# tspooner/rl_markets

Measured on AMD Instinct MI355X. Metric: env-steps/sec (whole node) at 65 536 parallel books, higher is better.
Workload: dtype f64

## Files before the change

### rl_markets_amd/csrc/lob_engine.hip

```cpp
#define LOB_TU_SPLIT 1
#define LOB_TU_MAIN 1
#include <hip/hip_runtime.h>
#include <math.h>
#include <stdio.h>
#include <stdlib.h>
#include <string.h>

#include <algorithm>
#include <climits>
#include <condition_variable>
#include <initializer_list>
#include <map>
#include <mutex>
#include <string>
#include <system_error>
#include <thread>
#include <vector>

#include "lob_internal.h"
#include "lob_fast.h"
#include "lob_kernels.h"
#include "lob_launch.h"

#define HIPCHK(expr)                                                                         \
// ... 8 lines not shown
#define LOB_PS(e) (const DevParams*)(e)->P_dev, (e)->S.self

#define LOB_HINT_RING 64
#define LOB_HINT_LAG 16
#define LOB_HINT_EVERY 8

struct KTimer {
    std::vector<std::pair<hipEvent_t, hipEvent_t>> pending;
    double total_ms = 0.0;
    int64_t launches = 0;
};

struct Switches {
    bool no_memo = false, no_carry = false, no_combine = false, light = true, force_fuse_act = false, t_light = true, no_fuse = false;
    bool q_pair = true, dq_pair = true, trace_lanes_off = false, acc_fuse = true, rest_merge = true, acc_dense = true;
    int q_lanes = -1, force_general = -1;
    int env_lanes = 0, env16_max = 4096;
    int acc_batches = 0, acc_shift = -1;
    int cb_slots = 0, ow_slots = 0, amb_cap = 0, cbd_ids = 0;
    int track_ring = 4096, track_refill = 64;
    long long upload_piece_recs = 0, spx_count = 0;
    bool upload_pinned = true;
    bool fuse_act = true, inline_general = true, env_step = true, prepass_roles = false, sarsa_lanes_off = false, dq_fast_off = false;
    bool rest_side = true, acc_block = true, exp_learn_first = false, no_hint = false;
    int env_step_lanes = 64, reset_lanes = 64, n_groups = 1, acc_reps = 0, ts_lds = 0, ts_grid = 0;
};

struct EnginePlan {
    int groups = 1;
    bool combine = false, memo = false, carry_verdicts = false, sarsa_lanes = false;
    bool q_lanes = false;
    bool q_pair = false;
    bool t_light = false;
    bool fuse = false;
    bool fused_act_ok = false;
    bool env_step = false, half_waves = false, env16 = false;
    bool inline_ok = false;
    int env_lanes = 64;
    bool acc_block_ok = false;
    bool dense_ids = false;
    bool acc_fuse_ok = false;
    bool rest_side_ok = false;
    bool learn_first = false;
};

struct lob_engine {
    int device = 0;
    int B = 0;
    lob_params params;
    Switches sw;
    EnginePlan plan;
    DevParams P;
    DevParams* P_dev = nullptr;
    DevState S;
    DevState* S_dev = nullptr;
    DevState S_pushed;
    hipStream_t stream = nullptr;
    hipStream_t stream2 = nullptr;
    hipEvent_t ev_fork = nullptr, ev_join = nullptr, ev_stagger = nullptr;
    hipEvent_t ev_rest_go = nullptr, ev_rest_done = nullptr;
    long long flow[8] = {0, 0, 0, 0, 0, 0, 0, 0};
    long long hint_reads = 0, hint_misses = 0;
    bool dense_ever = false;
    u64* rest_hint = nullptr;
    u64* rest_hint_dev = nullptr;
    hipEvent_t hint_ev[LOB_HINT_RING] = {};
    long long hint_step = 0;
    unsigned long long hint_serial = 0;
    uint32_t hint_tags[LOB_HINT_RING] = {};
    int hint_now = 0;
    int rest_recent = 0;
    int reg_apar = 0;
    int td_parity = 0;
    int step_id = 0;
    int list_par = 0;
    int last_par = 0;
// ... 178 lines not shown
bool env_is(const char* n, char c) { const char* g = getenv(n); return g && g[0] == c; }
long long env_in(const char* n, long long lo, long long hi, long long dflt) { const char* g = getenv(n); const long long v = g ? atoll(g) : dflt; return v >= lo && v <= hi ? v : dflt; }
int env_one_of(const char* n, std::initializer_list<int> allowed, int dflt) {
    const char* g = getenv(n);
    for (int a : allowed) if (g && atoi(g) == a) return a;
    return dflt;
}
int env_pow2(const char* n, int lo, int hi, int dflt) { const int v = (int)env_in(n, lo, hi, dflt); return (v & (v - 1)) == 0 ? v : dflt; }

Switches read_switches() {
    Switches s;
    s.no_memo = env_is("LOB_NO_MEMO", '1'); s.no_carry = env_is("LOB_NO_CARRY", '1'); s.no_combine = env_is("LOB_NO_COMBINE", '1');
    s.light = !env_is("LOB_NO_LIGHT", '1'); s.force_fuse_act = env_is("LOB_FUSE_ACT", '1');
    s.t_light = !env_is("LOB_NO_TLIGHT", '1'); s.no_fuse = env_is("LOB_NO_FUSE", '1');
    s.q_pair = !env_is("LOB_Q_PAIR", '0'); s.dq_pair = !env_is("LOB_DQ_PAIR", '0'); s.trace_lanes_off = env_is("LOB_TRACE_LANES", '0');
    s.acc_fuse = !env_is("LOB_ACC_FUSE", '0'); s.rest_merge = !env_is("LOB_REST_MERGE", '0'); s.acc_dense = !env_is("LOB_ACC_DENSE", '0');
    s.q_lanes = env_set("LOB_Q_LANES") ? (env_is("LOB_Q_LANES", '1') ? 1 : 0) : -1;
    s.force_general = env_is("LOB_MOSTLY_GENERAL", '1') ? 1 : env_is("LOB_MOSTLY_GENERAL", '0') ? 0 : -1;
    const bool exps = lobk_experiments() != 0;
    s.env_lanes = exps ? env_one_of("LOB_ENV_LANES", {16, 32, 64, 256}, 0) : env_one_of("LOB_ENV_LANES", {16, 64}, 0);
    s.env16_max = (int)env_in("LOB_ENV16_MAX", 0, INT_MAX, s.env16_max);
    s.acc_batches = env_one_of("LOB_ACC_BATCHES", {1, 2, 4, 8}, 0);
    const int acc_lanes = env_one_of("LOB_ACC_LANES", {8, 16, 32, 64}, 0);
    s.acc_shift = acc_lanes ? __builtin_ctz(acc_lanes) : -1;
    s.cb_slots = env_pow2("LOB_CB_SLOTS", 64, 1 << 24, 0); s.ow_slots = env_pow2("LOB_OW_SLOTS", 64, 1 << 26, 0);
    s.amb_cap = (int)env_in("LOB_AMB_CAP", 1, 1 << 18, 0); s.cbd_ids = (int)env_in("LOB_CBD_IDS", 8, LOB_CBD_CAP, 0);
    s.track_ring = env_pow2("LOB_TRACK_RING", 256, 1 << 20, s.track_ring); s.track_refill = (int)env_in("LOB_TRACK_REFILL", 1, INT_MAX, s.track_refill);
    s.upload_piece_recs = env_in("LOB_UPLOAD_PIECE_RECS", 1, LLONG_MAX, 0); s.upload_pinned = !env_is("LOB_UPLOAD_PINNED", '0');
    s.spx_count = env_in("LOB_SPX_COUNT", 64, LLONG_MAX, 0);
    if (!exps) return s;
// ... 6 lines not shown
    s.ts_lds = (int)env_in("LOB_TS_LDS", INT_MIN, INT_MAX, 0); s.ts_grid = (int)env_in("LOB_TS_GRID", INT_MIN, INT_MAX, 0);
    return s;
}

EnginePlan plan_paths(const DevParams& P, int B, int n_cus, const Switches& sw) {
    EnginePlan pl;
    const bool sarsa = P.algo == LOB_ALGO_SARSA, ql = P.algo == LOB_ALGO_QLAMBDA, dq = P.algo == LOB_ALGO_DOUBLE_Q;
    pl.groups = B >= 1024 ? sw.n_groups : 1;
    pl.combine = !P.theta_private && !sw.no_combine;
    pl.env_lanes = sw.env_lanes ? sw.env_lanes : (B <= 16384 ? 16 : 64);
    pl.fused_act_ok = sw.light && sw.fuse_act && sw.env_lanes == 0 && (B >= 1024 || sw.force_fuse_act);
    pl.env_step = P.T <= 2 && sw.env_step;
    pl.half_waves = sw.env_step_lanes == 32 && pl.env_step && !dq;
    pl.inline_ok = pl.env_step && sw.inline_general && !pl.half_waves;
    pl.env16 = !dq && B <= sw.env16_max && P.D <= 16 && P.Wd <= 64;
    pl.q_lanes = sw.q_lanes >= 0 ? sw.q_lanes == 1 : (long long)B >= (long long)LOB_QL_BLOCK * n_cus / 2;
    pl.q_pair = sw.q_pair && P.M < (1ll << 27) && (!dq || sw.dq_pair);
    pl.t_light = (ql || dq) && sw.t_light;
    pl.fuse = pl.t_light && pl.q_lanes && !sw.no_fuse;
    pl.memo = !P.theta_private && !P.r_learn && sw.n_groups == 1 && !sw.no_memo;
    if (dq) pl.memo = pl.memo && pl.fuse && pl.fused_act_ok && pl.env_step && pl.combine && P.trace_gens == 32 && !sw.dq_fast_off;
    pl.carry_verdicts = !P.theta_private && !sw.no_carry && !pl.memo;
    pl.sarsa_lanes = pl.memo && pl.combine && P.trace_gens == 32 && !sw.sarsa_lanes_off && !sw.trace_lanes_off && (sarsa || pl.fuse);
    pl.acc_block_ok = sw.acc_block && pl.memo && B >= 4 * LOB_ACB_BLOCK;
    pl.dense_ids = pl.acc_block_ok && pl.combine && sw.acc_dense && (sarsa || ql) && P.trace_gens <= LOB_TRACE_GENS;
    pl.acc_fuse_ok = pl.fuse && sw.acc_fuse && pl.combine && pl.sarsa_lanes && (ql || dq) && pl.groups == 1;
    pl.rest_side_ok = pl.fuse && sw.rest_side;
    pl.learn_first = sw.exp_learn_first && sarsa;
    return pl;
}
// ... 952 lines not shown
}

struct StepPlan {
    bool first, second;
    int mode;
    bool learner, fast;
    int par, lpar;
    u64 ver;
    bool acc_blocked, dense_on;
    int acc_shift;
    bool fused_act, mostly_general, inline_general;
    bool acc_fused;
    bool rest_merged;
    bool rest_side;
    bool registered;
};

struct StepGroup {
    int g, b0, nb;
    hipStream_t st;
    int gw, gf, gl;
};
static StepGroup step_group(const lob_engine* e, int g, int G) {
    const int b0 = (int)((long long)e->B * g / G), nb = (int)((long long)e->B * (g + 1) / G) - b0;
    return {g, b0, nb, g == 0 ? e->stream : e->stream2, grid_waves(nb),
            std::min(e->n_cus, (nb + LOB_FAST_WAVES * LOB_FAST_NB - 1) / (LOB_FAST_WAVES * LOB_FAST_NB)), 2 * e->n_cus};
}

static int read_hint(lob_engine* e, const StepPlan& sp) {
    e->hint_now = 0;
// ... 30 lines not shown
    if (sp.first) e->step_id++;
    if (!e->hits_ok) e->steps_on_lists = 0;
    sp.ver = (u64)e->theta_ver;
    if (sp.first) { const int rc = read_hint(e, sp); if (rc) return rc; }
    sp.lpar = sp.first ? (e->list_par ^= 1) : e->list_par;
    e->last_par = sp.par;
    const bool greedy = e->P.policy == LOB_POLICY_EPS_GREEDY && e->P.epsilon < 0.34;
    sp.acc_blocked = pl.acc_block_ok && (e->P.algo == LOB_ALGO_SARSA || (e->P.algo == LOB_ALGO_QLAMBDA && greedy));
    sp.dense_on = e->S.cb_dense && sp.acc_blocked;
    sp.acc_shift = e->sw.acc_shift >= 0 ? e->sw.acc_shift : (e->P.algo == LOB_ALGO_SARSA && e->S.cb_reps > 1) || greedy ? 6 : 5;
    if (sp.first) {
        sp.fused_act = sp.fast && sp.learner && e->hits_ok && pl.fused_act_ok;
        sp.mostly_general = e->sw.force_general >= 0 ? e->sw.force_general == 1 : e->hint_now > e->B / 16;
        sp.inline_general = pl.inline_ok && e->steps_on_lists >= 1 && !sp.mostly_general;
        if (sp.fused_act) e->steps_on_lists++;
    }
    if (sp.second && sp.learner && sp.fast) {
        sp.acc_fused = pl.acc_fuse_ok && !sp.acc_blocked && e->hint_now <= std::max(1024, e->B / 16);
        sp.rest_merged = sp.acc_fused && e->sw.rest_merge;
        if (!sp.rest_merged) {
            if (e->hint_now > 0) e->rest_recent = 64;
            else if (e->rest_recent > 0) e->rest_recent--;
            sp.rest_side = pl.rest_side_ok && e->rest_recent > 0;
        }
    }
    sp.registered = sp.second && sp.learner && e->P.sarsa_lanes;
    return LOB_OK;
}

static void count_flow(lob_engine* e, const StepPlan& sp, int half) {
    if (half == 1) { e->flow[sp.inline_general ? 4 : sp.mostly_general ? 5 : 6]++; return; }
    e->flow[sp.acc_blocked ? 2 : sp.acc_fused ? 0 : 3]++;
    if (sp.dense_on) e->flow[7]++;
    if (sp.rest_side) e->flow[1]++;
}

static int set_step_words(lob_engine* e, const StepPlan& sp) {
    if (sp.learner) e->S.cb_par = sp.par;
    if (sp.dense_on) e->dense_ever = true;
    if (sp.dense_on && !e->S.cb_dense_on) HIPCHK(hipMemsetAsync(e->S.tr_cbd, 0xff, (size_t)e->B * e->P.trace_gens * 8, e->stream));
    e->S.cb_dense_on = sp.dense_on;
    return LOB_OK;
}
static void publish_step_words(lob_engine* e, const StepPlan& sp, hipStream_t st) {
    if (sp.fast) launch_memo(e, sp.par, sp.learner ? 0 : 1);
    else if (sp.learner && e->P.combine) hipLaunchKernelGGL(step_words_kernel, dim3(1), dim3(1), 0, st, e->S_dev, e->S.cb_par, e->S.cb_dense_on);
}

static int act_half(lob_engine* e, const StepPlan& sp, const StepGroup& gr, int G) {
    const hipStream_t st = gr.st;
    const uint32_t* rnd = (const uint32_t*)e->rnd_dev;
    const bool dq = e->P.algo == LOB_ALGO_DOUBLE_Q;
    const i32* act_list = e->S.slow_list, *act_n = e->S.slow_n + sp.lpar * 2;
    if (G > 1 && gr.g == 1) HIPCHK(hipStreamWaitEvent(st, e->ev_stagger, 0));
    if (sp.fused_act) {
        count_flow(e, sp, 1);
        const DevParams* Pd = (const DevParams*)e->P_dev;
        const bool t2 = e->P.T <= 2;
        const int nb = e->B, sid = e->step_id;
        const EnvFuse F1{nullptr, nullptr, sp.lpar, sid - 1, sp.ver}, F2{act_list, act_n, sp.lpar, sid - 1, sp.ver};
        {
            TimedLaunch t(e, "env_kernel", st);
            if (e->plan.env_step) lobk_env_step(st, sp.inline_general, dq, e->plan.half_waves, e->plan.env16, Pd, e->S, nb, sid, sp.par, F1, rnd);
            else lobk_env_mode(st, t2, 1, Pd, e->S, nb, sid, sp.par, F1);
        }
        if (!sp.inline_general) {
            {
                TimedLaunch t(e, "act_rest_kernel", st);
                if (dq) hipLaunchKernelGGL((act_kernel<LOB_ALGO_DOUBLE_Q, true>), dim3(gr.gl), dim3(LOB_BLOCK), 0, st, LOB_PS(e), rnd, 0, 0, e->B, sp.par, act_list, act_n);
                else hipLaunchKernelGGL((act_kernel<LOB_ALGO_SARSA, true>), dim3(gr.gl), dim3(LOB_BLOCK), 0, st, LOB_PS(e), rnd, 0, 0, e->B, sp.par, act_list, act_n);
            }
            TimedLaunch t(e, "env_rest_kernel", st);
            lobk_env_mode(st, t2, 2, Pd, e->S, nb, sid, sp.par, F2);
        }
    } else if (sp.fast && !dq) {
        {
            TimedLaunch t(e, "act_kernel", st);
            if (sp.learner && e->hits_ok && e->sw.light)
// ... 688 lines not shown
}

extern "C" int lob_debug_light(lob_engine* e, int64_t out[2]) {
    if (!e || !out) return LOB_EINVAL;
    HIPCHK(hipSetDevice(e->device));
    i64 c[16];
    i32 d = 0;
    { int rc = read_counters(e, c); if (rc) return rc; }
    HIPCHK(hipMemcpyAsync(&d, e->S.hl_dirty, sizeof d, hipMemcpyDeviceToHost, e->stream));
    HIPCHK(hipStreamSynchronize(e->stream));
    out[0] = c[5];
    out[1] = d;
    return LOB_OK;
}

extern "C" int lob_debug_exchange(lob_engine* e, int64_t out[5]) {
    if (!e || !out) return LOB_EINVAL;
    out[0] = e->spx_nosync; out[1] = e->spx_synced; out[2] = e->spx_overflows; out[3] = e->spx_fixed; out[4] = e->spx_last_total;
    return LOB_OK;
}

extern "C" int lob_debug_deferred(lob_engine* e, int64_t out[1]) {
    if (!e || !out) return LOB_EINVAL;
    HIPCHK(hipSetDevice(e->device));
    i64 c[16];
    { int rc = read_counters(e, c); if (rc) return rc; }
    HIPCHK(hipStreamSynchronize(e->stream));
    out[0] = c[8];
    return LOB_OK;
}
// ... 19 lines not shown
```

### rl_markets_amd/csrc/lob_envstep.h

```cpp
#ifndef LOB_ENVSTEP_H
#define LOB_ENVSTEP_H

#include "lob_fast.h"

__device__ inline Track track_load(const Track* p) {
    const uint4* q = reinterpret_cast<const uint4*>(p);
    uint4 w[8];
#pragma unroll
    for (int i = 0; i < 8; i++) w[i] = q[i];
    Track t;
    uint4* d = reinterpret_cast<uint4*>(&t);
#pragma unroll
    for (int i = 0; i < 8; i++) d[i] = w[i];
    return t;
}

template <int LANES> struct EnvStepOcc { static constexpr int waves = LANES == 64 ? 1 : 2; };
template <bool INLINE_GENERAL, bool DQ = false, int LANES = 64>
__global__ void __launch_bounds__(64, EnvStepOcc<LANES>::waves) env_step_kernel(const DevParams* __restrict__ Pp, const DevState* __restrict__ Sp, int step_id, int par, EnvFuse F,
                                                                                  const uint32_t* __restrict__ rnd_g) {
    static_assert(LANES == 64 || !INLINE_GENERAL, "the half-full variant leaves the books without a list to the work list");
    const DevParams& P = *Pp;
    const DevState& S = *Sp;
    __shared__ TickLds tick_lds;
    __shared__ EnvSlot lds_env[LANES == 64 ? 64 : LANES + 1];
    __shared__ LearnLds1 lds_learn;
#ifdef LOB_PROF
    const long long t_entry = clock64();
#else
    const long long t_entry = 0;
#endif
    const int t = blockIdx.x * LANES + (int)threadIdx.x;
    const bool valid = (int)threadIdx.x < LANES && t < S.B;
    const int b = valid ? t : S.B - 1;
    const int B = S.B;

// ... 81 lines not shown
    RowFull cur, first;
    row_full_load(c, rc0, cur);
    {
        const int last_row = S.events_of(b) - 1;
        row_full_load(c, rc0 + 1 < last_row ? rc0 + 1 : last_row, first);
    }
    rm_prep(S.pnl_ups, B, b, wu);
    rm_prep(S.pnl_downs, B, b, wd);
#ifdef LOB_PROF
    __builtin_amdgcn_s_waitcnt(0);
    const long long t_r2 = clock64();
#endif

    int action = 0;
    bool go = false;
    if (valid) {
        if (h0.done) {
            hp->stepped = 0;
        } else if (!open) {
            hp->slot_cur = cur_slot; hp->done = 1; hp->stepped = 0; S.done[b] = 1;
        } else {
            ok = ok && rec.ver == F.ver;
            if (!ok) {
                if (!INLINE_GENERAL) {
                    const int pos = atomicAdd(&S.slow_n[F.lpar * 2 + 0], 1);
                    S.slow_list[pos] = b;
                }
            } else {
                f64 q[LOB_N_ACTIONS];
#pragma unroll
// ... 62 lines not shown
                    }
#pragma unroll
                    for (int a = 0; a < LOB_N_ACTIONS; a++) {
                        S.qs_last_b[(size_t)b * LOB_N_ACTIONS + a] = qb[a];
                        q[a] = (q[a] + qb[a]) / 2.0;
                    }
                }
                Rng g{P.seed, P.book_id_offset + (u64)b, h0.rng_ctr};
                action = policy_sample(P, q, false, g);
                hp->slot_cur = cur_slot;
                hp->action = action;
                hp->stepped = 1;
                hp->rng_ctr = g.ctr;
                const uint32_t marked = tiles_ok ? mk_bits : 0x1ffu;
                if (!((marked >> action) & 1u)) {
                    const int pos = atomicAdd(&S.mk_markcount[0], 1);
                    if (pos < S.mk_slots) S.mk_marklist[pos] = mslot * 16 + action;
                    else mark_generation(P, S, mslot, action);
                    atomicOr(&S.mk_marked[mslot], 1u << action);
                }
                const u64 act = __ballot(1);
                if ((int)(threadIdx.x & 63) == __builtin_ctzll(act)) cnt_add(S, 5, (unsigned long long)__builtin_popcountll(act));
                go = true;
            }
        }
    }
#undef LOB_HL_ENT
    if (INLINE_GENERAL) {
        u64 todo = __ballot(valid && alive && open && !ok);
        if (todo) {
            if (threadIdx.x == 0) cnt_add(S, 2, (u64)__builtin_popcountll(todo));
            const uint4* src = reinterpret_cast<const uint4*>(rnd_g);
            uint4* dst = reinterpret_cast<uint4*>(lds_learn.rnd);
            for (int i = threadIdx.x; i < 512; i += 64) dst[i] = src[i];
            if (threadIdx.x < 27) lds_learn.act_terms[threadIdx.x] = rnd_g[2048 + threadIdx.x];
            wave_lds_fence();
            while (todo) {
                const int src_lane = __builtin_ctzll(todo);
                todo &= todo - 1;
                const int b_src = __builtin_amdgcn_readlane(b, src_lane);
                int act = -1;
                act_book<DQ ? LOB_ALGO_DOUBLE_Q : LOB_ALGO_SARSA, LearnLds1>(P, S, lds_learn, 0, (int)threadIdx.x, b_src, 0, par, &act);
                if ((int)threadIdx.x == src_lane && act >= 0) { action = act; go = true; }
            }
        }
    }

    i64 d_steps = 0, d_events = 0;
    if (go) {
        c.pre_prev = &tprev;
        c.pre_n_track = m_n_track;
// ... 34 lines not shown
            }
            hp->zero_mask = h0.zero_mask & ~(1 << cs);
            S.verdict[(size_t)b * LOB_VD_STRIDE + 67] = 0;
            hp->reward = get_reward(c, e, &tcur.spread_mean);
            hp->stepped = 1;
            d_steps = 1;
        } else {
            hp->stepped = 0;
        }
        c.mark(28);
        hp->done = e.done;
        hp->time_ms = e.time_ms;
        env_store(S, b, e);
        if (claim) {
            S.mk_slot_last[b] = claim_slot_prev;
            S.mk_slot[b] = mk_claim(S, claim_q0, claim_q1, claim_q2, step_id, par, claim_k, claim_stamp);
        }
        c.mark(29);
        c.flush();
    }
    for (int off = 32; off > 0; off >>= 1) {
        d_steps += __shfl_down(d_steps, off);
        d_events += __shfl_down(d_events, off);
    }
    if ((threadIdx.x & 63) == 0 && (d_steps | d_events)) {
        cnt_add(S, 0, (u64)d_steps);
        cnt_add(S, 1, (u64)d_events);
        cnt_add(S, 3, (u64)d_steps);
    }
}


#define LOB_ENV16_BOOKS 4
static_assert(LOB_HL_MAX <= 48, "env_step16_kernel gathers a hit list in three 16-lane loads");
// ... 217 lines not shown
```

### rl_markets_amd/csrc/lob_kernels.h

```cpp
#ifndef LOB_KERNELS_H
#define LOB_KERNELS_H

#include <hip/hip_runtime.h>

#include "lob_state.h"
#include "lob_stream.h"
#include "lob_launch.h"
#include "lob_stats.h"

#if !defined(LOB_TU_SPLIT)
#define LOB_IN_MAIN 1
#define LOB_IN_ENV 1
#define LOB_IN_PREPASS 1
#define LOB_IN_STATS 1
#else
#if defined(LOB_TU_STATS)
#define LOB_IN_STATS 1
#else
#define LOB_IN_STATS 0
#endif
#if defined(LOB_TU_MAIN)
#define LOB_IN_MAIN 1
#else
#define LOB_IN_MAIN 0
// ... 1933 lines not shown
    const int s_first = S.mk_list[(size_t)par * S.mk_slots + (wave < S.mk_slots ? wave : 0)];
    int count = S.mk_count[par];
    {
        const uint4* src = reinterpret_cast<const uint4*>(rnd_g);
        uint4* dst = reinterpret_cast<uint4*>(rnd);
        const uint4 r0 = src[threadIdx.x], r1 = src[threadIdx.x + 256];
        dst[threadIdx.x] = r0; dst[threadIdx.x + 256] = r1;
        if (threadIdx.x < 27) rnd[2048 + threadIdx.x] = rnd_g[2048 + threadIdx.x];
    }
    __syncthreads();
    if (count > S.mk_slots) count = S.mk_slots;
    f64* v = vals[w];
    for (int i = wave; i < count; i += n_waves) {
        const int s = i == wave ? s_first : S.mk_list[(size_t)par * S.mk_slots + i];
        const int4 id = *reinterpret_cast<const int4*>(S.mk_ident + (size_t)s * 4);
        uint32_t sum = 0;
        {
            int base = j;
            sum = mod_add(sum, rnd[(tile_coord(id.x, base) + 449 * 0) & 2047], M); base += 2 * j;
            sum = mod_add(sum, rnd[(tile_coord(id.y, base) + 449 * 1) & 2047], M); base += 2 * j;
            sum = mod_add(sum, rnd[(tile_coord(id.z, base) + 449 * 2) & 2047], M);
            sum = mod_add(sum, rnd[(j + 449 * 3) & 2047], M);
        }
        f64 t[5], tb[5];
        const bool fill = (S.mk_tiles_ok[s] & 1) == 0;
        const bool two = S.mk_rec_b != nullptr;
        if (which == 0 && !fill) {
            const f64* r1 = S.mk_rec + ((size_t)S.mk_slots + s) * LOB_MK_REC;
            if (reinterpret_cast<const u64*>(r1)[LOB_N_ACTIONS] == ver) {
                f64* r0 = S.mk_rec + (size_t)s * LOB_MK_REC;
                if (lane <= LOB_N_ACTIONS) reinterpret_cast<u64*>(r0)[lane] = reinterpret_cast<const u64*>(r1)[lane];
                if (two) {
                    const f64* b1 = S.mk_rec_b + ((size_t)S.mk_slots + s) * LOB_MK_REC;
                    f64* b0 = S.mk_rec_b + (size_t)s * LOB_MK_REC;
                    if (lane <= LOB_N_ACTIONS) reinterpret_cast<u64*>(b0)[lane] = reinterpret_cast<const u64*>(b1)[lane];
                }
                continue;
            }
        }
#pragma unroll
        for (int k = 0; k < 5; k++) {
            const int a = (hi ? 5 : 0) + k;
            const i32 tile = tile_index(sum, rnd[2048 + (a < LOB_N_ACTIONS ? a : 0)], M);
            t[k] = a < LOB_N_ACTIONS ? S.theta[tile] : 0.0;
            tb[k] = (two && a < LOB_N_ACTIONS) ? S.theta_b[tile] : 0.0;
            if (fill && a < LOB_N_ACTIONS) S.mk_tiles[((size_t)s * LOB_N_ACTIONS + a) * 32 + j] = tile;
        }
        if (fill && lane == 0) {
            __threadfence();
            atomicOr(&S.mk_tiles_ok[s], 1);
        }
#pragma unroll
        for (int k = 0; k < 5; k++) {
            const int a = (hi ? 5 : 0) + k;
            if (a < LOB_N_ACTIONS) v[a * LOB_QSTRIDE + j] = P.w0 * t[k];
        }
        __builtin_amdgcn_fence(__ATOMIC_ACQ_REL, "workgroup", "local");
        __builtin_amdgcn_wave_barrier();
        f64 q = 0.0;
        if (lane < LOB_N_ACTIONS) {
            for (int k = 0; k < 32; k++) q += v[lane * LOB_QSTRIDE + k];
        }
        f64* rec = S.mk_rec + ((size_t)which * S.mk_slots + s) * LOB_MK_REC;
        if (lane < LOB_N_ACTIONS) rec[lane] = q;
        if (lane == LOB_N_ACTIONS) reinterpret_cast<u64*>(rec)[LOB_N_ACTIONS] = ver;
        __builtin_amdgcn_fence(__ATOMIC_ACQ_REL, "workgroup", "local");
        __builtin_amdgcn_wave_barrier();
        if (two) {
#pragma unroll
            for (int k = 0; k < 5; k++) {
                const int a = (hi ? 5 : 0) + k;
                if (a < LOB_N_ACTIONS) v[a * LOB_QSTRIDE + j] = P.w0 * tb[k];
            }
            __builtin_amdgcn_fence(__ATOMIC_ACQ_REL, "workgroup", "local");
            __builtin_amdgcn_wave_barrier();
            f64 qb = 0.0;
            if (lane < LOB_N_ACTIONS) {
                for (int k = 0; k < 32; k++) qb += v[lane * LOB_QSTRIDE + k];
            }
            f64* recb = S.mk_rec_b + ((size_t)which * S.mk_slots + s) * LOB_MK_REC;
            if (lane < LOB_N_ACTIONS) recb[lane] = qb;
            if (lane == LOB_N_ACTIONS) reinterpret_cast<u64*>(recb)[LOB_N_ACTIONS] = ver;
            __builtin_amdgcn_fence(__ATOMIC_ACQ_REL, "workgroup", "local");
            __builtin_amdgcn_wave_barrier();
        }
    }
    if (which == 0) {
        int nm = S.mk_markcount[0];
        if (nm > S.mk_slots) nm = S.mk_slots;
        for (int i = wave; i < nm; i += n_waves) {
            const int e = S.mk_marklist[i];
            if (lane < 32) nzx_mark(P, S, S.mk_tiles[((size_t)(e >> 4) * LOB_N_ACTIONS + (e & 15)) * 32 + lane]);
        }
    } else if (blockIdx.x == 0 && threadIdx.x == 0) {
        S.mk_markcount[0] = 0;
    }
}
#endif

#if LOB_IN_MAIN
// ... 497 lines not shown
```

### rl_markets_amd/csrc/lob_launch.h

```cpp
#ifndef LOB_LAUNCH_H
#define LOB_LAUNCH_H

#include <hip/hip_runtime.h>

#include "lob_state.h"

struct EnvFuse {
    const i32* list;
    const i32* list_n;
    int lpar, sid_prev;
    u64 ver;
};

int lobk_experiments();

void lobk_env(hipStream_t st, int lanes, bool t2, const DevParams* Pd, const DevState& S, const i32* actions, int count_updates, int b0, int nb, int sid, int par);
void lobk_env_mode(hipStream_t st, bool t2, int mode, const DevParams* Pd, const DevState& S, int nb, int sid, int par, const EnvFuse& F);
void lobk_env_step(hipStream_t st, bool inline_general, bool dq, bool half_waves, bool lanes16, const DevParams* Pd, const DevState& S, int nb, int sid, int par,
                   const EnvFuse& F, const uint32_t* rnd);
void lobk_clear_inventory(hipStream_t st, const DevParams* Pd, const DevState& S);
void lobk_get_state(hipStream_t st, const DevParams* Pd, const DevState& S, f32* out, f64* reward);
void lobk_dump(hipStream_t st, const DevParams* Pd, const DevState& S, int first, int n, lob_book_dump* out);

void lobk_gen_events(hipStream_t st, const lob_gen_params& g, int D, int T, u64 first_book, int B, uint32_t* out);
void lobk_repack(hipStream_t st, const uint32_t* src, int D, int T, size_t n_records, uint32_t* dst);
void lobk_days_draw(hipStream_t st, int B, u64 first_book, int mode, int first, int n, const i32* explicit_day, uint32_t* rng, const i64* day_first,
                    const i32* day_len, i64* rec_phase, i32* rec_len, i32* day);
void lobk_reset(hipStream_t st, int lanes, bool t2, bool roles, const DevParams* Pd, const DevState& S);
void lobk_prepass_extend(hipStream_t st, bool t2, bool roles, const DevParams* Pd, const DevState& S);
void lobk_finalize(hipStream_t st, bool t2, const DevParams* Pd, const DevState& S);

#define LOB_STATS_BLOCK 256
#define LOB_STATS_CHUNK 2048
struct StatsSrc {
// ... 18 lines not shown
```

### rl_markets_amd/csrc/lob_learn.h

```cpp
#ifndef LOB_LEARN_H
#define LOB_LEARN_H

#include <hip/hip_runtime.h>

#include "lob_state.h"
#include "lob_stream.h"
#include "lob_exp_table.h"

#ifdef LOB_PROF
struct Prof {
    long long t;
    i64* row;
    __device__ void start(i64* prof, int book, int lane) { row = (prof && lane == 0) ? prof + (size_t)book * LOB_PROF_N : nullptr; t = clock64(); }
    __device__ void mark(int i) {
        const long long n = clock64();
        if (row) row[i] += n - t;
        t = n;
    }
};
#else
struct Prof {
    __device__ void start(i64*, int, int) {}
    __device__ void mark(int) {}
};
// ... 292 lines not shown
        for (int i = 0; i < 32; i++) q += col[i];
    }
#pragma unroll
    for (int a = 0; a < LOB_N_ACTIONS; a++) out_q[a] = __shfl(q, a);
    __builtin_amdgcn_fence(__ATOMIC_ACQ_REL, "workgroup", "local");
    __builtin_amdgcn_wave_barrier();
}


#define LOB_MK_EMPTY (~0ull)
__device__ inline u64 mk_hash3(int q0, int q1, int q2) {
    u64 h = lob_mix64((u64)(uint32_t)q0 | ((u64)(uint32_t)q1 << 32));
    h = lob_mix64(h + (u64)(uint32_t)q2 * 0x9E3779B97F4A7C15ull);
    return h == LOB_MK_EMPTY ? 0 : h;
}
__device__ inline int mk_claim(const DevState& S, int q0, int q1, int q2, int step_id, int par, u64 pre_k, int pre_stamp) {
    const u64 h = mk_hash3(q0, q1, q2);
    const uint32_t mask = (uint32_t)(S.mk_slots - 1);
    uint32_t s = (uint32_t)h & mask;
    if (pre_k == h && pre_stamp == step_id) return (int)s;
    for (int probe = 0; probe < LOB_MK_PROBES; probe++) {
        u64 k = probe == 0 ? pre_k : S.mk_hash[s];
        if (k == LOB_MK_EMPTY) {
            k = atomicCAS((unsigned long long*)&S.mk_hash[s], (unsigned long long)LOB_MK_EMPTY, (unsigned long long)h);
            if (k == LOB_MK_EMPTY) {
                *reinterpret_cast<int4*>(S.mk_ident + (size_t)s * 4) = make_int4(q0, q1, q2, 0);
                k = h;
            }
        }
        if (k == h) {
            if (S.mk_stamp[s] != step_id) {
                const int old = atomicExch(&S.mk_stamp[s], step_id);
                if (old != step_id) {
                    const int pos = atomicAdd(&S.mk_count[par], 1);
                    if (pos < S.mk_slots) S.mk_list[(size_t)par * S.mk_slots + pos] = (i32)s;
                }
            }
            return (int)s;
        }
        s = (s + 1) & mask;
    }
    return -1;
}

__device__ inline f64 readlane_f64(f64 x, int l) {
    const int lo = __builtin_amdgcn_readlane(__double2loint(x), l);
    const int hi = __builtin_amdgcn_readlane(__double2hiint(x), l);
    return __hiloint2double(hi, lo);
}

struct MemoRec {
    f64 s0[LOB_N_ACTIONS];
    u64 ver;
};
static_assert(sizeof(MemoRec) == LOB_MK_REC * 8, "memo record layout");

#define LOB_MT_N 312
#define LOB_MT_M 156
__host__ __device__ inline void mt64_seed(u64* x, u64 seed) {
    x[0] = seed;
    for (int i = 1; i < LOB_MT_N; i++) x[i] = 6364136223846793005ull * (x[i - 1] ^ (x[i - 1] >> 62)) + (u64)i;
}
__host__ __device__ inline u64 mt64_mix(u64 xi, u64 xi1, u64 xm) {
    const u64 y = (xi & 0xFFFFFFFF80000000ull) | (xi1 & 0x7FFFFFFFull);
    return xm ^ (y >> 1) ^ ((y & 1ull) ? 0xB5026F5AA96619E9ull : 0ull);
}
__device__ inline void mt64_twist_wave(u64* gstate, u64* lds, int lane) {
    for (int i = lane; i < LOB_MT_N; i += 64) lds[i] = gstate[i];
    __builtin_amdgcn_fence(__ATOMIC_ACQ_REL, "workgroup", "local");
    __builtin_amdgcn_wave_barrier();
// ... 51 lines not shown
```

### rl_markets_amd/csrc/lob_tu_env.hip

```cpp
#define LOB_TU_SPLIT 1
#define LOB_TU_ENV 1
#include <hip/hip_runtime.h>

#include "lob_internal.h"
#include "lob_fast.h"
#include "lob_kernels.h"
#include "lob_envstep.h"

int lobk_experiments() {
#ifdef LOB_EXPERIMENTS
    return 1;
#else
    return 0;
#endif
}

void lobk_env(hipStream_t st, int lanes, bool t2, const DevParams* Pd, const DevState& S, const i32* actions, int count_updates, int b0, int nb, int sid, int par) {
#define LOB_ENV_LAUNCH(L, TM) hipLaunchKernelGGL((env_kernel<L, TM>), dim3((nb + L - 1) / L), dim3(L), 0, st, Pd, S, actions, count_updates, b0, nb, sid, par)
#ifdef LOB_EXPERIMENTS
    if (!actions && lanes == 256) {
        hipLaunchKernelGGL(env_compact_kernel, dim3((nb + LOB_ENVC_BLOCK - 1) / LOB_ENVC_BLOCK), dim3(LOB_ENVC_BLOCK), 0, st, Pd, S, count_updates, b0, nb, sid, par);
        return;
    }
    if (lanes == 32) { if (t2) LOB_ENV_LAUNCH(32, 2); else LOB_ENV_LAUNCH(32, LOB_MAX_TRADES); return; }
// ... 2 lines not shown
    else { if (t2) LOB_ENV_LAUNCH(64, 2); else LOB_ENV_LAUNCH(64, LOB_MAX_TRADES); }
#undef LOB_ENV_LAUNCH
}

void lobk_env_mode(hipStream_t st, bool t2, int mode, const DevParams* Pd, const DevState& S, int nb, int sid, int par, const EnvFuse& F) {
    const dim3 grid((nb + 63) / 64), block(64);
    if (mode == 1) {
        if (t2) hipLaunchKernelGGL((env_kernel<64, 2, 1>), grid, block, 0, st, Pd, S, (const i32*)nullptr, 1, 0, nb, sid, par, F);
        else hipLaunchKernelGGL((env_kernel<64, LOB_MAX_TRADES, 1>), grid, block, 0, st, Pd, S, (const i32*)nullptr, 1, 0, nb, sid, par, F);
    } else {
        if (t2) hipLaunchKernelGGL((env_kernel<64, 2, 2>), grid, block, 0, st, Pd, S, (const i32*)nullptr, 1, 0, nb, sid, par, F);
        else hipLaunchKernelGGL((env_kernel<64, LOB_MAX_TRADES, 2>), grid, block, 0, st, Pd, S, (const i32*)nullptr, 1, 0, nb, sid, par, F);
    }
}

void lobk_env_step(hipStream_t st, bool inline_general, bool dq, bool half_waves, bool lanes16, const DevParams* Pd, const DevState& S, int nb, int sid, int par,
                   const EnvFuse& F, const uint32_t* rnd) {
    const dim3 grid((nb + 63) / 64), block(64);
    if (lanes16 && !dq) {
        const dim3 g16((nb + LOB_ENV16_BOOKS - 1) / LOB_ENV16_BOOKS);
        if (inline_general) hipLaunchKernelGGL(env_step16_kernel<true>, g16, block, 0, st, Pd, S.self, sid, par, F, rnd);
        else hipLaunchKernelGGL(env_step16_kernel<false>, g16, block, 0, st, Pd, S.self, sid, par, F, rnd);
        return;
    }
#define LOB_S_ARG S.self
#ifdef LOB_EXPERIMENTS
    if (half_waves && !dq && !inline_general) {
        hipLaunchKernelGGL((env_step_kernel<false, false, 32>), dim3((nb + 31) / 32), block, 0, st, Pd, LOB_S_ARG, sid, par, F, rnd);
        return;
    }
#endif
    (void)half_waves;
    if (inline_general && dq) hipLaunchKernelGGL((env_step_kernel<true, true>), grid, block, 0, st, Pd, LOB_S_ARG, sid, par, F, rnd);
    else if (dq) hipLaunchKernelGGL((env_step_kernel<false, true>), grid, block, 0, st, Pd, LOB_S_ARG, sid, par, F, rnd);
    else if (inline_general) hipLaunchKernelGGL(env_step_kernel<true>, grid, block, 0, st, Pd, LOB_S_ARG, sid, par, F, rnd);
    else hipLaunchKernelGGL(env_step_kernel<false>, grid, block, 0, st, Pd, LOB_S_ARG, sid, par, F, rnd);
#undef LOB_S_ARG
}

void lobk_clear_inventory(hipStream_t st, const DevParams* Pd, const DevState& S) {
    hipLaunchKernelGGL(clear_inventory_kernel, dim3((S.B + 255) / 256), dim3(256), 0, st, Pd, S);
}
void lobk_get_state(hipStream_t st, const DevParams* Pd, const DevState& S, f32* out, f64* reward) {
    hipLaunchKernelGGL(get_state_kernel, dim3((S.B + 255) / 256), dim3(256), 0, st, Pd, S, out, reward);
}
void lobk_dump(hipStream_t st, const DevParams* Pd, const DevState& S, int first, int n, lob_book_dump* out) {
    hipLaunchKernelGGL(dump_kernel, dim3((n + 63) / 64), dim3(64), 0, st, Pd, S, first, n, out);
}
// ... 1 lines not shown
```

Before: 287.8 million.

## Fuse memo evaluation and mark publishing into the env-step kernel tail

Adds a MEMO_TAIL variant of env_step_kernel. Each lane that wins a memo-slot claim copies the slot's record forward when its version is current, and otherwise evaluates the slot in-wave through a new shared memo_eval_slot helper. Marked tiles go straight to nzx_mark instead of through the mark list, and the separate memo launch in publish_step_words is skipped for such steps. This removes a kernel launch and a pass over the claim list per step, at the cost of serialized per-wave evaluation loops and extra register and LDS pressure in the env kernel. It is on by default and can be disabled with LOB_MEMO_LAUNCH=1.

```diff
diff --git a/rl_markets_amd/csrc/lob_engine.hip b/rl_markets_amd/csrc/lob_engine.hip
--- a/rl_markets_amd/csrc/lob_engine.hip
+++ b/rl_markets_amd/csrc/lob_engine.hip
@@ -46,6 +46,7 @@
 struct Switches {
     bool no_memo = false, no_carry = false, no_combine = false, light = true, force_fuse_act = false, t_light = true, no_fuse = false;
     bool q_pair = true, dq_pair = true, trace_lanes_off = false, acc_fuse = true, rest_merge = true, acc_dense = true;
+    bool memo_launch = false;
     int q_lanes = -1, force_general = -1;
     int env_lanes = 0, env16_max = 4096;
     int acc_batches = 0, acc_shift = -1;
@@ -68,6 +69,7 @@
     bool fused_act_ok = false;
     bool env_step = false, half_waves = false, env16 = false;
     bool inline_ok = false;
+    bool memo_tail_ok = false;
     int env_lanes = 64;
     bool acc_block_ok = false;
     bool dense_ids = false;
@@ -92,6 +94,7 @@
     hipEvent_t ev_fork = nullptr, ev_join = nullptr, ev_stagger = nullptr;
     hipEvent_t ev_rest_go = nullptr, ev_rest_done = nullptr;
     long long flow[8] = {0, 0, 0, 0, 0, 0, 0, 0};
+    long long memo_tail_steps = 0;
     long long hint_reads = 0, hint_misses = 0;
     bool dense_ever = false;
     u64* rest_hint = nullptr;
@@ -300,6 +303,7 @@
     s.light = !env_is("LOB_NO_LIGHT", '1'); s.force_fuse_act = env_is("LOB_FUSE_ACT", '1');
     s.t_light = !env_is("LOB_NO_TLIGHT", '1'); s.no_fuse = env_is("LOB_NO_FUSE", '1');
     s.q_pair = !env_is("LOB_Q_PAIR", '0'); s.dq_pair = !env_is("LOB_DQ_PAIR", '0'); s.trace_lanes_off = env_is("LOB_TRACE_LANES", '0');
+    s.memo_launch = env_is("LOB_MEMO_LAUNCH", '1');
     s.acc_fuse = !env_is("LOB_ACC_FUSE", '0'); s.rest_merge = !env_is("LOB_REST_MERGE", '0'); s.acc_dense = !env_is("LOB_ACC_DENSE", '0');
     s.q_lanes = env_set("LOB_Q_LANES") ? (env_is("LOB_Q_LANES", '1') ? 1 : 0) : -1;
     s.force_general = env_is("LOB_MOSTLY_GENERAL", '1') ? 1 : env_is("LOB_MOSTLY_GENERAL", '0') ? 0 : -1;
@@ -336,6 +340,7 @@
     pl.half_waves = sw.env_step_lanes == 32 && pl.env_step && !dq;
     pl.inline_ok = pl.env_step && sw.inline_general && !pl.half_waves;
     pl.env16 = !dq && B <= sw.env16_max && P.D <= 16 && P.Wd <= 64;
+    pl.memo_tail_ok = !sw.memo_launch && pl.env_step && lobk_env_step_has_memo_tail(pl.inline_ok, dq, pl.half_waves, pl.env16);
     pl.q_lanes = sw.q_lanes >= 0 ? sw.q_lanes == 1 : (long long)B >= (long long)LOB_QL_BLOCK * n_cus / 2;
     pl.q_pair = sw.q_pair && P.M < (1ll << 27) && (!dq || sw.dq_pair);
     pl.t_light = (ql || dq) && sw.t_light;
@@ -1318,6 +1323,7 @@
     bool rest_merged;
     bool rest_side;
     bool registered;
+    bool memo_tail;
 };
 
 struct StepGroup {
@@ -1378,6 +1384,8 @@
         sp.mostly_general = e->sw.force_general >= 0 ? e->sw.force_general == 1 : e->hint_now > e->B / 16;
         sp.inline_general = pl.inline_ok && e->steps_on_lists >= 1 && !sp.mostly_general;
         if (sp.fused_act) e->steps_on_lists++;
+        sp.memo_tail = pl.memo_tail_ok && pl.memo && sp.second && sp.fused_act && sp.inline_general;
+        if (sp.memo_tail) e->memo_tail_steps++;
     }
     if (sp.second && sp.learner && sp.fast) {
         sp.acc_fused = pl.acc_fuse_ok && !sp.acc_blocked && e->hint_now <= std::max(1024, e->B / 16);
@@ -1407,6 +1415,7 @@
     return LOB_OK;
 }
 static void publish_step_words(lob_engine* e, const StepPlan& sp, hipStream_t st) {
+    if (sp.memo_tail) return;
     if (sp.fast) launch_memo(e, sp.par, sp.learner ? 0 : 1);
     else if (sp.learner && e->P.combine) hipLaunchKernelGGL(step_words_kernel, dim3(1), dim3(1), 0, st, e->S_dev, e->S.cb_par, e->S.cb_dense_on);
 }
@@ -1422,10 +1431,10 @@
         const DevParams* Pd = (const DevParams*)e->P_dev;
         const bool t2 = e->P.T <= 2;
         const int nb = e->B, sid = e->step_id;
-        const EnvFuse F1{nullptr, nullptr, sp.lpar, sid - 1, sp.ver}, F2{act_list, act_n, sp.lpar, sid - 1, sp.ver};
+        const EnvFuse F1{nullptr, nullptr, sp.lpar, sid - 1, sp.ver, e->S.cb_dense_on}, F2{act_list, act_n, sp.lpar, sid - 1, sp.ver, e->S.cb_dense_on};
         {
             TimedLaunch t(e, "env_kernel", st);
-            if (e->plan.env_step) lobk_env_step(st, sp.inline_general, dq, e->plan.half_waves, e->plan.env16, Pd, e->S, nb, sid, sp.par, F1, rnd);
+            if (e->plan.env_step) lobk_env_step(st, sp.inline_general, dq, e->plan.half_waves, e->plan.env16, sp.memo_tail, Pd, e->S, nb, sid, sp.par, F1, rnd);
             else lobk_env_mode(st, t2, 1, Pd, e->S, nb, sid, sp.par, F1);
         }
         if (!sp.inline_general) {
@@ -2144,6 +2153,46 @@
     return LOB_OK;
 }
 
+extern "C" int lob_debug_memo_array(lob_engine* e, int32_t which, void* out, int64_t cap, int64_t* n_bytes) {
+    if (!e || !n_bytes) return LOB_EINVAL;
+    if (!e->P.memo) { lob_set_error("lob_debug_memo_array: the engine runs without the group-0 memo"); return LOB_ESTATE; }
+    HIPCHK(hipSetDevice(e->device));
+    const size_t ms = (size_t)e->S.mk_slots, mw = (size_t)e->P.M / 32 + 1;
+    const void* src = nullptr;
+    size_t n = 0;
+    if (which == 10) {
+        *n_bytes = 8;
+        if (out && cap >= 8) *(int64_t*)out = e->memo_tail_steps;
+        return LOB_OK;
+    }
+    switch (which) {
+    case 0: {
+        i32 cnt[2] = {0, 0};
+        HIPCHK(hipMemcpyAsync(cnt, e->S.mk_count, sizeof cnt, hipMemcpyDeviceToHost, e->stream));
+        HIPCHK(hipStreamSynchronize(e->stream));
+        const int par = e->last_par & 1;
+        src = e->S.mk_list + (size_t)par * ms; n = (size_t)std::min<i64>(std::max(cnt[par], 0), (i64)ms) * 4;
+        break;
+    }
+    case 1: src = e->S.mk_ident; n = ms * 16; break;
+    case 2: src = e->S.mk_rec; n = 2 * ms * LOB_MK_REC * 8; break;
+    case 3: src = e->S.mk_rec_b; n = e->S.mk_rec_b ? 2 * ms * LOB_MK_REC * 8 : 0; break;
+    case 4: src = e->S.mk_tiles; n = ms * LOB_N_ACTIONS * 32 * 4; break;
+    case 5: src = e->S.mk_tiles_ok; n = ms * 4; break;
+    case 6: src = e->S.theta_nzx; n = mw * 4; break;
+    case 7: src = e->S.theta_nzc; n = (size_t)e->P.cwords4 * 16; break;
+    case 8: src = e->S.theta_nzd; n = e->S.theta_nzd ? 2 * mw * 4 : 0; break;
+    case 9: src = e->S.hl_rec; n = (size_t)LOB_HL_REC * e->B * 8; break;
+    default: lob_set_error("lob_debug_memo_array: unknown array"); return LOB_EINVAL;
+    }
+    *n_bytes = (int64_t)n;
+    if (!out || n == 0) return LOB_OK;
+    if (cap < (int64_t)n) { lob_set_error("lob_debug_memo_array: the buffer is too small"); return LOB_EINVAL; }
+    HIPCHK(hipMemcpyAsync(out, src, n, hipMemcpyDeviceToHost, e->stream));
+    HIPCHK(hipStreamSynchronize(e->stream));
+    return LOB_OK;
+}
+
 extern "C" int lob_debug_exchange(lob_engine* e, int64_t out[5]) {
     if (!e || !out) return LOB_EINVAL;
     out[0] = e->spx_nosync; out[1] = e->spx_synced; out[2] = e->spx_overflows; out[3] = e->spx_fixed; out[4] = e->spx_last_total;
diff --git a/rl_markets_amd/csrc/lob_envstep.h b/rl_markets_amd/csrc/lob_envstep.h
--- a/rl_markets_amd/csrc/lob_envstep.h
+++ b/rl_markets_amd/csrc/lob_envstep.h
@@ -16,10 +16,11 @@
 }
 
 template <int LANES> struct EnvStepOcc { static constexpr int waves = LANES == 64 ? 1 : 2; };
-template <bool INLINE_GENERAL, bool DQ = false, int LANES = 64>
+template <bool INLINE_GENERAL, bool DQ = false, int LANES = 64, bool MEMO_TAIL = false>
 __global__ void __launch_bounds__(64, EnvStepOcc<LANES>::waves) env_step_kernel(const DevParams* __restrict__ Pp, const DevState* __restrict__ Sp, int step_id, int par, EnvFuse F,
                                                                                   const uint32_t* __restrict__ rnd_g) {
     static_assert(LANES == 64 || !INLINE_GENERAL, "the half-full variant leaves the books without a list to the work list");
+    static_assert(!MEMO_TAIL || (INLINE_GENERAL && LANES == 64), "the memo tail serves the step whose claims are all made by this kernel");
     const DevParams& P = *Pp;
     const DevState& S = *Sp;
     __shared__ TickLds tick_lds;
@@ -131,6 +132,10 @@
 
     int action = 0;
     bool go = false;
+    int mark_pair = -1;
+    int won = 0, won_slot = 0;
+    int won_q0 = 0, won_q1 = 0, won_q2 = 0;
+    bool rnd_staged = false;
     if (valid) {
         if (h0.done) {
             hp->stepped = 0;
@@ -223,9 +228,13 @@
                 hp->rng_ctr = g.ctr;
                 const uint32_t marked = tiles_ok ? mk_bits : 0x1ffu;
                 if (!((marked >> action) & 1u)) {
-                    const int pos = atomicAdd(&S.mk_markcount[0], 1);
-                    if (pos < S.mk_slots) S.mk_marklist[pos] = mslot * 16 + action;
-                    else mark_generation(P, S, mslot, action);
+                    if (MEMO_TAIL) {
+                        mark_pair = mslot * 16 + action;
+                    } else {
+                        const int pos = atomicAdd(&S.mk_markcount[0], 1);
+                        if (pos < S.mk_slots) S.mk_marklist[pos] = mslot * 16 + action;
+                        else mark_generation(P, S, mslot, action);
+                    }
                     atomicOr(&S.mk_marked[mslot], 1u << action);
                 }
                 const u64 act = __ballot(1);
@@ -244,6 +253,7 @@
             for (int i = threadIdx.x; i < 512; i += 64) dst[i] = src[i];
             if (threadIdx.x < 27) lds_learn.act_terms[threadIdx.x] = rnd_g[2048 + threadIdx.x];
             wave_lds_fence();
+            rnd_staged = true;
             while (todo) {
                 const int src_lane = __builtin_ctzll(todo);
                 todo &= todo - 1;
@@ -308,10 +318,71 @@
         env_store(S, b, e);
         if (claim) {
             S.mk_slot_last[b] = claim_slot_prev;
-            S.mk_slot[b] = mk_claim(S, claim_q0, claim_q1, claim_q2, step_id, par, claim_k, claim_stamp);
+            const int ns = mk_claim(S, claim_q0, claim_q1, claim_q2, step_id, par, claim_k, claim_stamp, MEMO_TAIL ? &won : nullptr);
+            S.mk_slot[b] = ns;
+            if (MEMO_TAIL) { won_slot = ns; won_q0 = claim_q0; won_q1 = claim_q1; won_q2 = claim_q2; }
         }
         c.mark(29);
         c.flush();
+    }
+    if (MEMO_TAIL) {
+        if (blockIdx.x == 0 && threadIdx.x == 0) {
+            DevState* w = const_cast<DevState*>(Sp);
+            w->cb_par = par;
+            w->cb_dense_on = F.dense_on;
+        }
+        const int lane = (int)threadIdx.x;
+        const bool two = S.mk_rec_b != nullptr;
+        bool eval = false;
+        if (won) {
+            const u64* r1 = reinterpret_cast<const u64*>(S.mk_rec + ((size_t)S.mk_slots + won_slot) * LOB_MK_REC);
+            const int okb = S.mk_tiles_ok[won_slot];
+            u64 w1[LOB_MK_REC], wb[LOB_MK_REC];
+#pragma unroll
+            for (int i = 0; i < LOB_MK_REC; i++) w1[i] = r1[i];
+            if (two) {
+                const u64* b1 = reinterpret_cast<const u64*>(S.mk_rec_b + ((size_t)S.mk_slots + won_slot) * LOB_MK_REC);
+#pragma unroll
+                for (int i = 0; i < LOB_MK_REC; i++) wb[i] = b1[i];
+            }
+            if ((okb & 1) && w1[LOB_N_ACTIONS] == F.ver) {
+                u64* r0 = reinterpret_cast<u64*>(S.mk_rec + (size_t)won_slot * LOB_MK_REC);
+#pragma unroll
+                for (int i = 0; i < LOB_MK_REC; i++) r0[i] = w1[i];
+                if (two) {
+                    u64* b0 = reinterpret_cast<u64*>(S.mk_rec_b + (size_t)won_slot * LOB_MK_REC);
+#pragma unroll
+                    for (int i = 0; i < LOB_MK_REC; i++) b0[i] = wb[i];
+                }
+            } else {
+                eval = true;
+            }
+        }
+        u64 todo = __ballot(eval);
+        if (todo) {
+            if (!rnd_staged) {
+                const uint4* src = reinterpret_cast<const uint4*>(rnd_g);
+                uint4* dst = reinterpret_cast<uint4*>(lds_learn.rnd);
+                for (int i = threadIdx.x; i < 512; i += 64) dst[i] = src[i];
+                if (threadIdx.x < 27) lds_learn.act_terms[threadIdx.x] = rnd_g[2048 + threadIdx.x];
+            }
+            wave_lds_fence();
+            while (todo) {
+                const int src_lane = __builtin_ctzll(todo);
+                todo &= todo - 1;
+                const int s = __builtin_amdgcn_readlane(won_slot, src_lane);
+                const int q0 = __builtin_amdgcn_readlane(won_q0, src_lane), q1 = __builtin_amdgcn_readlane(won_q1, src_lane), q2 = __builtin_amdgcn_readlane(won_q2, src_lane);
+                const bool fill = (S.mk_tiles_ok[s] & 1) == 0;
+                memo_eval_slot(P, S, lds_learn.rnd, lds_learn.act_terms, lds_learn.vals[0], lane, s, q0, q1, q2, 0, F.ver, fill, two);
+            }
+        }
+        u64 mm = __ballot(mark_pair >= 0);
+        while (mm) {
+            const int src_lane = __builtin_ctzll(mm);
+            mm &= mm - 1;
+            const int e = __builtin_amdgcn_readlane(mark_pair, src_lane);
+            if (lane < 32) nzx_mark(P, S, S.mk_tiles[((size_t)(e >> 4) * LOB_N_ACTIONS + (e & 15)) * 32 + lane]);
+        }
     }
     for (int off = 32; off > 0; off >>= 1) {
         d_steps += __shfl_down(d_steps, off);
diff --git a/rl_markets_amd/csrc/lob_kernels.h b/rl_markets_amd/csrc/lob_kernels.h
--- a/rl_markets_amd/csrc/lob_kernels.h
+++ b/rl_markets_amd/csrc/lob_kernels.h
@@ -1971,15 +1971,6 @@
     for (int i = wave; i < count; i += n_waves) {
         const int s = i == wave ? s_first : S.mk_list[(size_t)par * S.mk_slots + i];
         const int4 id = *reinterpret_cast<const int4*>(S.mk_ident + (size_t)s * 4);
-        uint32_t sum = 0;
-        {
-            int base = j;
-            sum = mod_add(sum, rnd[(tile_coord(id.x, base) + 449 * 0) & 2047], M); base += 2 * j;
-            sum = mod_add(sum, rnd[(tile_coord(id.y, base) + 449 * 1) & 2047], M); base += 2 * j;
-            sum = mod_add(sum, rnd[(tile_coord(id.z, base) + 449 * 2) & 2047], M);
-            sum = mod_add(sum, rnd[(j + 449 * 3) & 2047], M);
-        }
-        f64 t[5], tb[5];
         const bool fill = (S.mk_tiles_ok[s] & 1) == 0;
         const bool two = S.mk_rec_b != nullptr;
         if (which == 0 && !fill) {
@@ -1995,52 +1986,7 @@
                 continue;
             }
         }
-#pragma unroll
-        for (int k = 0; k < 5; k++) {
-            const int a = (hi ? 5 : 0) + k;
-            const i32 tile = tile_index(sum, rnd[2048 + (a < LOB_N_ACTIONS ? a : 0)], M);
-            t[k] = a < LOB_N_ACTIONS ? S.theta[tile] : 0.0;
-            tb[k] = (two && a < LOB_N_ACTIONS) ? S.theta_b[tile] : 0.0;
-            if (fill && a < LOB_N_ACTIONS) S.mk_tiles[((size_t)s * LOB_N_ACTIONS + a) * 32 + j] = tile;
-        }
-        if (fill && lane == 0) {
-            __threadfence();
-            atomicOr(&S.mk_tiles_ok[s], 1);
-        }
-#pragma unroll
-        for (int k = 0; k < 5; k++) {
-            const int a = (hi ? 5 : 0) + k;
-            if (a < LOB_N_ACTIONS) v[a * LOB_QSTRIDE + j] = P.w0 * t[k];
-        }
-        __builtin_amdgcn_fence(__ATOMIC_ACQ_REL, "workgroup", "local");
-        __builtin_amdgcn_wave_barrier();
-        f64 q = 0.0;
-        if (lane < LOB_N_ACTIONS) {
-            for (int k = 0; k < 32; k++) q += v[lane * LOB_QSTRIDE + k];
-        }
-        f64* rec = S.mk_rec + ((size_t)which * S.mk_slots + s) * LOB_MK_REC;
-        if (lane < LOB_N_ACTIONS) rec[lane] = q;
-        if (lane == LOB_N_ACTIONS) reinterpret_cast<u64*>(rec)[LOB_N_ACTIONS] = ver;
-        __builtin_amdgcn_fence(__ATOMIC_ACQ_REL, "workgroup", "local");
-        __builtin_amdgcn_wave_barrier();
-        if (two) {
-#pragma unroll
-            for (int k = 0; k < 5; k++) {
-                const int a = (hi ? 5 : 0) + k;
-                if (a < LOB_N_ACTIONS) v[a * LOB_QSTRIDE + j] = P.w0 * tb[k];
-            }
-            __builtin_amdgcn_fence(__ATOMIC_ACQ_REL, "workgroup", "local");
-            __builtin_amdgcn_wave_barrier();
-            f64 qb = 0.0;
-            if (lane < LOB_N_ACTIONS) {
-                for (int k = 0; k < 32; k++) qb += v[lane * LOB_QSTRIDE + k];
-            }
-            f64* recb = S.mk_rec_b + ((size_t)which * S.mk_slots + s) * LOB_MK_REC;
-            if (lane < LOB_N_ACTIONS) recb[lane] = qb;
-            if (lane == LOB_N_ACTIONS) reinterpret_cast<u64*>(recb)[LOB_N_ACTIONS] = ver;
-            __builtin_amdgcn_fence(__ATOMIC_ACQ_REL, "workgroup", "local");
-            __builtin_amdgcn_wave_barrier();
-        }
+        memo_eval_slot(P, S, rnd, rnd + 2048, v, lane, s, id.x, id.y, id.z, which, ver, fill, two);
     }
     if (which == 0) {
         int nm = S.mk_markcount[0];
diff --git a/rl_markets_amd/csrc/lob_launch.h b/rl_markets_amd/csrc/lob_launch.h
--- a/rl_markets_amd/csrc/lob_launch.h
+++ b/rl_markets_amd/csrc/lob_launch.h
@@ -10,14 +10,16 @@
     const i32* list_n;
     int lpar, sid_prev;
     u64 ver;
+    int dense_on;
 };
 
 int lobk_experiments();
 
 void lobk_env(hipStream_t st, int lanes, bool t2, const DevParams* Pd, const DevState& S, const i32* actions, int count_updates, int b0, int nb, int sid, int par);
 void lobk_env_mode(hipStream_t st, bool t2, int mode, const DevParams* Pd, const DevState& S, int nb, int sid, int par, const EnvFuse& F);
-void lobk_env_step(hipStream_t st, bool inline_general, bool dq, bool half_waves, bool lanes16, const DevParams* Pd, const DevState& S, int nb, int sid, int par,
-                   const EnvFuse& F, const uint32_t* rnd);
+void lobk_env_step(hipStream_t st, bool inline_general, bool dq, bool half_waves, bool lanes16, bool memo_tail, const DevParams* Pd, const DevState& S, int nb,
+                   int sid, int par, const EnvFuse& F, const uint32_t* rnd);
+inline bool lobk_env_step_has_memo_tail(bool inline_general, bool dq, bool half_waves, bool lanes16) { return inline_general && !half_waves && !(lanes16 && !dq); }
 void lobk_clear_inventory(hipStream_t st, const DevParams* Pd, const DevState& S);
 void lobk_get_state(hipStream_t st, const DevParams* Pd, const DevState& S, f32* out, f64* reward);
 void lobk_dump(hipStream_t st, const DevParams* Pd, const DevState& S, int first, int n, lob_book_dump* out);
diff --git a/rl_markets_amd/csrc/lob_learn.h b/rl_markets_amd/csrc/lob_learn.h
--- a/rl_markets_amd/csrc/lob_learn.h
+++ b/rl_markets_amd/csrc/lob_learn.h
@@ -330,7 +330,7 @@
     h = lob_mix64(h + (u64)(uint32_t)q2 * 0x9E3779B97F4A7C15ull);
     return h == LOB_MK_EMPTY ? 0 : h;
 }
-__device__ inline int mk_claim(const DevState& S, int q0, int q1, int q2, int step_id, int par, u64 pre_k, int pre_stamp) {
+__device__ inline int mk_claim(const DevState& S, int q0, int q1, int q2, int step_id, int par, u64 pre_k, int pre_stamp, int* won = nullptr) {
     const u64 h = mk_hash3(q0, q1, q2);
     const uint32_t mask = (uint32_t)(S.mk_slots - 1);
     uint32_t s = (uint32_t)h & mask;
@@ -349,7 +349,10 @@
                 const int old = atomicExch(&S.mk_stamp[s], step_id);
                 if (old != step_id) {
                     const int pos = atomicAdd(&S.mk_count[par], 1);
-                    if (pos < S.mk_slots) S.mk_list[(size_t)par * S.mk_slots + pos] = (i32)s;
+                    if (pos < S.mk_slots) {
+                        S.mk_list[(size_t)par * S.mk_slots + pos] = (i32)s;
+                        if (won) *won = 1;
+                    }
                 }
             }
             return (int)s;
@@ -370,6 +373,68 @@
     u64 ver;
 };
 static_assert(sizeof(MemoRec) == LOB_MK_REC * 8, "memo record layout");
+
+__device__ __forceinline__ void memo_eval_slot(const DevParams& P, const DevState& S, const uint32_t* rnd, const uint32_t* terms, f64* v, int lane,
+                                               int s, int q0, int q1, int q2, int which, u64 ver, bool fill, bool two) {
+    const int j = lane & 31;
+    const bool hi = lane >= 32;
+    const uint32_t M = (uint32_t)P.M;
+    uint32_t sum = 0;
+    {
+        int base = j;
+        sum = mod_add(sum, rnd[(tile_coord(q0, base) + 449 * 0) & 2047], M); base += 2 * j;
+        sum = mod_add(sum, rnd[(tile_coord(q1, base) + 449 * 1) & 2047], M); base += 2 * j;
+        sum = mod_add(sum, rnd[(tile_coord(q2, base) + 449 * 2) & 2047], M);
+        sum = mod_add(sum, rnd[(j + 449 * 3) & 2047], M);
+    }
+    f64 t[5], tb[5];
+#pragma unroll
+    for (int k = 0; k < 5; k++) {
+        const int a = (hi ? 5 : 0) + k;
+        const i32 tile = tile_index(sum, terms[a < LOB_N_ACTIONS ? a : 0], M);
+        t[k] = a < LOB_N_ACTIONS ? S.theta[tile] : 0.0;
+        tb[k] = (two && a < LOB_N_ACTIONS) ? S.theta_b[tile] : 0.0;
+        if (fill && a < LOB_N_ACTIONS) S.mk_tiles[((size_t)s * LOB_N_ACTIONS + a) * 32 + j] = tile;
+    }
+    if (fill && lane == 0) {
+        __threadfence();
+        atomicOr(&S.mk_tiles_ok[s], 1);
+    }
+#pragma unroll
+    for (int k = 0; k < 5; k++) {
+        const int a = (hi ? 5 : 0) + k;
+        if (a < LOB_N_ACTIONS) v[a * LOB_QSTRIDE + j] = P.w0 * t[k];
+    }
+    __builtin_amdgcn_fence(__ATOMIC_ACQ_REL, "workgroup", "local");
+    __builtin_amdgcn_wave_barrier();
+    f64 q = 0.0;
+    if (lane < LOB_N_ACTIONS) {
+        for (int k = 0; k < 32; k++) q += v[lane * LOB_QSTRIDE + k];
+    }
+    f64* rec = S.mk_rec + ((size_t)which * S.mk_slots + s) * LOB_MK_REC;
+    if (lane < LOB_N_ACTIONS) rec[lane] = q;
+    if (lane == LOB_N_ACTIONS) reinterpret_cast<u64*>(rec)[LOB_N_ACTIONS] = ver;
+    __builtin_amdgcn_fence(__ATOMIC_ACQ_REL, "workgroup", "local");
+    __builtin_amdgcn_wave_barrier();
+    if (two) {
+#pragma unroll
+        for (int k = 0; k < 5; k++) {
+            const int a = (hi ? 5 : 0) + k;
+            if (a < LOB_N_ACTIONS) v[a * LOB_QSTRIDE + j] = P.w0 * tb[k];
+        }
+        __builtin_amdgcn_fence(__ATOMIC_ACQ_REL, "workgroup", "local");
+        __builtin_amdgcn_wave_barrier();
+        f64 qb = 0.0;
+        if (lane < LOB_N_ACTIONS) {
+            for (int k = 0; k < 32; k++) qb += v[lane * LOB_QSTRIDE + k];
+        }
+        f64* recb = S.mk_rec_b + ((size_t)which * S.mk_slots + s) * LOB_MK_REC;
+        if (lane < LOB_N_ACTIONS) recb[lane] = qb;
+        if (lane == LOB_N_ACTIONS) reinterpret_cast<u64*>(recb)[LOB_N_ACTIONS] = ver;
+        __builtin_amdgcn_fence(__ATOMIC_ACQ_REL, "workgroup", "local");
+        __builtin_amdgcn_wave_barrier();
+    }
+}
 
 #define LOB_MT_N 312
 #define LOB_MT_M 156
diff --git a/rl_markets_amd/csrc/lob_tu_env.hip b/rl_markets_amd/csrc/lob_tu_env.hip
--- a/rl_markets_amd/csrc/lob_tu_env.hip
+++ b/rl_markets_amd/csrc/lob_tu_env.hip
@@ -40,8 +40,8 @@
     }
 }
 
-void lobk_env_step(hipStream_t st, bool inline_general, bool dq, bool half_waves, bool lanes16, const DevParams* Pd, const DevState& S, int nb, int sid, int par,
-                   const EnvFuse& F, const uint32_t* rnd) {
+void lobk_env_step(hipStream_t st, bool inline_general, bool dq, bool half_waves, bool lanes16, bool memo_tail, const DevParams* Pd, const DevState& S, int nb,
+                   int sid, int par, const EnvFuse& F, const uint32_t* rnd) {
     const dim3 grid((nb + 63) / 64), block(64);
     if (lanes16 && !dq) {
         const dim3 g16((nb + LOB_ENV16_BOOKS - 1) / LOB_ENV16_BOOKS);
@@ -57,7 +57,11 @@
     }
 #endif
     (void)half_waves;
-    if (inline_general && dq) hipLaunchKernelGGL((env_step_kernel<true, true>), grid, block, 0, st, Pd, LOB_S_ARG, sid, par, F, rnd);
+    if (memo_tail && inline_general) {
+        if (dq) hipLaunchKernelGGL((env_step_kernel<true, true, 64, true>), grid, block, 0, st, Pd, LOB_S_ARG, sid, par, F, rnd);
+        else hipLaunchKernelGGL((env_step_kernel<true, false, 64, true>), grid, block, 0, st, Pd, LOB_S_ARG, sid, par, F, rnd);
+    }
+    else if (inline_general && dq) hipLaunchKernelGGL((env_step_kernel<true, true>), grid, block, 0, st, Pd, LOB_S_ARG, sid, par, F, rnd);
     else if (dq) hipLaunchKernelGGL((env_step_kernel<false, true>), grid, block, 0, st, Pd, LOB_S_ARG, sid, par, F, rnd);
     else if (inline_general) hipLaunchKernelGGL(env_step_kernel<true>, grid, block, 0, st, Pd, LOB_S_ARG, sid, par, F, rnd);
     else hipLaunchKernelGGL(env_step_kernel<false>, grid, block, 0, st, Pd, LOB_S_ARG, sid, par, F, rnd);
```

Result: no change. 288.9 million (median of 3 runs) (+0.4%).
